# spacemeshos/go-spacemesh

Measured on AMD Instinct MI355X. Metric: post_labels_per_sec, higher is better.
Workload: dtype u32; 1 GPU; init-mainnet-scryptN8192-4units-256GiB-sink; step_labels=2097152, scrypt_n=8192, num_units=4, labels_per_unit=4294967296, parallelism=index-range shards x1, RCCL nonce min-reduce, vrf_nonce_found=True

## Files before the change

go-spacemesh_amd/csrc/engine.cpp:

```cpp
#include "../../include/spacemesh_post.h"

#include <hip/hip_runtime.h>

#include <fcntl.h>
#include <sys/stat.h>
#include <sys/types.h>
#include <unistd.h>

#include <algorithm>
#include <array>
#include <atomic>
#include <thread>
#include <chrono>
#include <cerrno>
#include <cstdio>
#include <cstdlib>
#include <cstring>
#include <functional>
#include <map>
#include <mutex>
#include <string>
#include <vector>

#include "crypto_host.h"
#include "kernel_args.h"
#include "post_common.h"

namespace {

thread_local std::string g_last_error;

void set_error(const std::string &e) { g_last_error = e; }

int hip_fail(const char *what, hipError_t err) {
  set_error(std::string(what) + ": " + hipGetErrorString(err));
  return err == hipErrorOutOfMemory ? POST_ERR_OOM : POST_ERR;
}

#define HIP_TRY(expr)                                                          \
  do {                                                                         \
    hipError_t _e = (expr);                                                    \
    if (_e != hipSuccess) return hip_fail(#expr, _e);                          \
  } while (0)

int require_gpu(uint32_t provider_id) {
  int count = 0;
  hipError_t e = hipGetDeviceCount(&count);
  if (e != hipSuccess || count == 0) {
    set_error("no HIP device available (the HIP engine has no CPU fallback)");
    return POST_ERR_NO_GPU;
  }
  if (provider_id >= (uint32_t)count) {
    set_error("provider id out of range");
    return POST_ERR_INVALID_ARGS;
  }
  e = hipSetDevice((int)provider_id);
  if (e != hipSuccess) return hip_fail("hipSetDevice", e);
  return POST_OK;
}

void load_commitment_words(const uint8_t c[32], uint32_t w[8]) {
  std::memcpy(w, c, 32);
}

void difficulty_to_be_words(const uint8_t d[32], uint32_t w[8]) {
  for (int i = 0; i < 8; i++)
    w[i] = ((uint32_t)d[4 * i] << 24) | ((uint32_t)d[4 * i + 1] << 16) |
           ((uint32_t)d[4 * i + 2] << 8) | d[4 * i + 3];
}

constexpr uint32_t THREADS = 256;
constexpr uint32_t CAND_CAP = 1 << 16;

uint32_t pick_gap_shift(uint32_t scrypt_n) {
  const char *env = getenv("POST_GAP_SHIFT");
  if (env) {
    uint32_t g = (uint32_t)atoi(env);
    while ((scrypt_n >> g) == 0) g--;
    return g;
  }
  return 0;
}

uint64_t prove_chunk_labels() {
  const uint64_t dflt = 1ull << 24;
  const char *env = getenv("POST_PROVE_CHUNK_LABELS");
  if (!env) return dflt;
  const long long v = strtoll(env, nullptr, 10);
  if (v <= 0 || (uint64_t)v >= dflt) return dflt;
  return v < 256 ? 256 : (uint64_t)v;
}

struct VerifyWorkspace {
  std::mutex mu;
  uint32_t *d_scratch = nullptr;
  size_t scratch_cap = 0;
  uint64_t *d_idx = nullptr;
  uint32_t *d_cid = nullptr;
  uint8_t *d_out = nullptr;
  uint32_t *d_xbuf = nullptr;
  size_t tasks_cap = 0;
  uint32_t *d_cm = nullptr;
  size_t cm_cap = 0;
  uint32_t *d_vrk = nullptr;
  uint8_t *d_half = nullptr;
  uint64_t *d_vdiff = nullptr;
  size_t proofs_cap = 0;
  uint8_t *d_pass = nullptr;
};
std::mutex g_vws_mu;
std::map<int, VerifyWorkspace *> g_vws;

VerifyWorkspace *get_verify_ws(int dev) {
  std::lock_guard<std::mutex> lk(g_vws_mu);
  auto it = g_vws.find(dev);
  if (it != g_vws.end()) return it->second;
  auto *w = new VerifyWorkspace();
  g_vws[dev] = w;
  return w;
}

int ws_reserve_proofs(VerifyWorkspace *w, size_t proofs) {
  if (proofs > w->proofs_cap) {
    size_t cap = std::max<size_t>(proofs, 1024);
    if (w->d_vrk) (void)hipFree(w->d_vrk);
    if (w->d_half) (void)hipFree(w->d_half);
    if (w->d_vdiff) (void)hipFree(w->d_vdiff);
    w->d_vrk = nullptr; w->d_half = nullptr; w->d_vdiff = nullptr;
    w->proofs_cap = 0;
    HIP_TRY(hipMalloc(&w->d_vrk, cap * 44 * 4));
    HIP_TRY(hipMalloc(&w->d_half, cap));
    HIP_TRY(hipMalloc(&w->d_vdiff, cap * 8));
    w->proofs_cap = cap;
  }
  return POST_OK;
}

int ws_reserve(VerifyWorkspace *w, size_t scratch_bytes, size_t tasks,
               size_t cm_words) {
  if (scratch_bytes > w->scratch_cap) {
    if (w->d_scratch) (void)hipFree(w->d_scratch);
    w->d_scratch = nullptr;
    w->scratch_cap = 0;
    HIP_TRY(hipMalloc(&w->d_scratch, scratch_bytes));
    w->scratch_cap = scratch_bytes;
  }
  if (tasks > w->tasks_cap) {
    size_t cap = std::max<size_t>(tasks, 4096);
    if (w->d_idx) (void)hipFree(w->d_idx);
    if (w->d_cid) (void)hipFree(w->d_cid);
    if (w->d_out) (void)hipFree(w->d_out);
    if (w->d_xbuf) (void)hipFree(w->d_xbuf);
    if (w->d_pass) (void)hipFree(w->d_pass);
    w->d_idx = nullptr; w->d_cid = nullptr; w->d_out = nullptr;
    w->d_xbuf = nullptr; w->d_pass = nullptr;
    w->tasks_cap = 0;
    HIP_TRY(hipMalloc(&w->d_idx, cap * 8));
    HIP_TRY(hipMalloc(&w->d_cid, cap * 4));
    HIP_TRY(hipMalloc(&w->d_out, cap * 32));
    HIP_TRY(hipMalloc(&w->d_xbuf, cap * 128));
    HIP_TRY(hipMalloc(&w->d_pass, cap));
    w->tasks_cap = cap;
  }
  if (cm_words > w->cm_cap) {
    size_t cap = std::max<size_t>(cm_words, 1024);
    if (w->d_cm) (void)hipFree(w->d_cm);
    w->d_cm = nullptr;
    w->cm_cap = 0;
    HIP_TRY(hipMalloc(&w->d_cm, cap * 4));
    w->cm_cap = cap;
  }
  return POST_OK;
}

struct DeviceTables {
  uint32_t *d_te = nullptr;
  uint8_t *d_sbox = nullptr;
};
std::mutex g_tables_mu;
std::map<int, DeviceTables> g_tables;

int get_aes_tables(int dev, DeviceTables &out) {
  std::lock_guard<std::mutex> lk(g_tables_mu);
  auto it = g_tables.find(dev);
  if (it != g_tables.end()) {
    out = it->second;
    return POST_OK;
  }
  static uint32_t te[1024];
  static uint8_t sbox[256];
  poste::aes128_tables(te, sbox);
  DeviceTables t;
  HIP_TRY(hipMalloc(&t.d_te, sizeof(te)));
  HIP_TRY(hipMalloc(&t.d_sbox, sizeof(sbox)));
  HIP_TRY(hipMemcpy(t.d_te, te, sizeof(te), hipMemcpyHostToDevice));
  HIP_TRY(hipMemcpy(t.d_sbox, sbox, sizeof(sbox), hipMemcpyHostToDevice));
  g_tables[dev] = t;
  out = t;
  return POST_OK;
}

}

extern "C" {

const char *post_last_error(void) { return g_last_error.c_str(); }

const char *post_engine_version(void) {
  return "spacemesh-post-hip 0.2 (gfx950)";
}


int post_providers(PostProvider *providers, uint32_t cap, uint32_t *count) {
  int n = 0;
  hipError_t e = hipGetDeviceCount(&n);
  if (e != hipSuccess) n = 0;
  *count = (uint32_t)n;
  for (uint32_t i = 0; i < (uint32_t)n && i < cap; i++) {
    hipDeviceProp_t prop;
    if (hipGetDeviceProperties(&prop, (int)i) != hipSuccess) continue;
    providers[i].id = i;
    std::snprintf(providers[i].model, sizeof(providers[i].model), "%s",
                  prop.name);
    providers[i].device_type = 0;
    providers[i].memory_bytes = prop.totalGlobalMem;
    providers[i].performance = 0;
  }
  return POST_OK;
}


struct PostInitSession {
  PostInitConfig cfg;
  std::string data_dir;
  uint64_t range_start = 0, range_end = 0;
  std::atomic<uint64_t> written{0};
  std::atomic<bool> cancel{false};
  uint8_t commitment[32];

  std::mutex nonce_mu;
  bool nonce_found = false;
  uint64_t nonce_idx = 0;
  uint8_t nonce_label[32];

  uint64_t lanes = 0;
  uint64_t batch_seq = 0;
  uint32_t gap_shift = 0;
  uint64_t batch = 0;
  uint32_t *d_scratch = nullptr;
  uint8_t *d_out = nullptr;
  uint8_t *d_all = nullptr;
  bool keep_all = false;
  PostVrfCandidate *d_cand = nullptr;
  unsigned int *d_cand_count = nullptr;
  uint32_t *d_xbuf = nullptr;
  uint8_t *h_batch = nullptr;
  hipStream_t stream = nullptr;
  hipEvent_t ev0 = nullptr, ev1 = nullptr;
  double last_kernel_ms = 0;

  int split_streams = 0;
  bool split_chain = false;
  uint64_t unit_cursor = 0;
  uint64_t split_batch_no = 0;
  uint32_t cand_cap = 0;
  uint8_t *d_out1 = nullptr;
  PostVrfCandidate *d_cand1 = nullptr;
  unsigned int *d_cand_count1 = nullptr;
  uint8_t *h_batch1 = nullptr;
  PostVrfCandidate *h_cand[2] = {nullptr, nullptr};
  unsigned int *h_cand_count = nullptr;
  hipStream_t stream_b = nullptr, stream_c = nullptr, copy_stream = nullptr;
  hipEvent_t ev_fill[4] = {nullptr, nullptr, nullptr, nullptr};
  hipEvent_t ev_tail[2][3] = {{nullptr, nullptr, nullptr},
                              {nullptr, nullptr, nullptr}};
  hipEvent_t ev_end[2] = {nullptr, nullptr}, ev_done[2] = {nullptr, nullptr};
  hipEvent_t ev_reset[2] = {nullptr, nullptr};

  ~PostInitSession() {
    if (stream) (void)hipStreamSynchronize(stream);
    if (stream_b) (void)hipStreamSynchronize(stream_b);
    if (stream_c) (void)hipStreamSynchronize(stream_c);
    if (copy_stream) (void)hipStreamSynchronize(copy_stream);
    for (int i = 0; i < 4; i++)
      if (ev_fill[i]) (void)hipEventDestroy(ev_fill[i]);
    for (int i = 0; i < 2; i++) {
      for (int k = 0; k < 3; k++)
        if (ev_tail[i][k]) (void)hipEventDestroy(ev_tail[i][k]);
      if (ev_reset[i]) (void)hipEventDestroy(ev_reset[i]);
      if (ev_end[i]) (void)hipEventDestroy(ev_end[i]);
      if (ev_done[i]) (void)hipEventDestroy(ev_done[i]);
      if (h_cand[i]) (void)hipHostFree(h_cand[i]);
    }
    if (stream_b) (void)hipStreamDestroy(stream_b);
    if (stream_c) (void)hipStreamDestroy(stream_c);
    if (copy_stream) (void)hipStreamDestroy(copy_stream);
    if (d_out1) (void)hipFree(d_out1);
    if (d_cand1) (void)hipFree(d_cand1);
    if (d_cand_count1) (void)hipFree(d_cand_count1);
    if (h_batch1) (void)hipHostFree(h_batch1);
    if (h_cand_count) (void)hipHostFree(h_cand_count);
    if (ev0) (void)hipEventDestroy(ev0);
    if (ev1) (void)hipEventDestroy(ev1);
    if (stream) (void)hipStreamDestroy(stream);
    if (d_scratch) (void)hipFree(d_scratch);
    if (d_out) (void)hipFree(d_out);
    if (d_all) (void)hipFree(d_all);
    if (d_cand) (void)hipFree(d_cand);
    if (d_cand_count) (void)hipFree(d_cand_count);
    if (d_xbuf) (void)hipFree(d_xbuf);
    if (h_batch) (void)hipHostFree(h_batch);
  }
};

static uint64_t existing_labels(const std::string &dir, uint64_t per_file,
                                uint64_t range_start, uint64_t range_total) {
  uint64_t done = 0;
  for (uint64_t pos = range_start; pos < range_start + range_total;) {
    uint64_t file_i = pos / per_file;
    uint64_t in_file = pos % per_file;
    uint64_t file_cap = std::min(per_file - in_file,
                                 range_start + range_total - pos);
    char path[4096];
    std::snprintf(path, sizeof path, "%s/postdata_%llu.bin", dir.c_str(),
                  (unsigned long long)file_i);
    FILE *f = std::fopen(path, "rb");
    if (!f) break;
    std::fseek(f, 0, SEEK_END);
    long sz = std::ftell(f);
    std::fclose(f);
    uint64_t labels_here = (uint64_t)(sz < 0 ? 0 : sz) / POST_LABEL_SIZE;
    if (in_file > labels_here) break;
    uint64_t usable = std::min(labels_here - in_file, file_cap);
    done += usable;
    pos += usable;
    if (usable < file_cap) break;
  }
  return done;
}

static int check_existing_metadata(PostInitSession *s);
static int write_metadata(PostInitSession *s);

int post_init_new(const PostInitConfig *cfg, PostInitSession **out) {
  if (!cfg || !out) {
    set_error("null args");
    return POST_ERR_INVALID_ARGS;
  }
  if (cfg->scrypt_n < 2 || (cfg->scrypt_n & (cfg->scrypt_n - 1))) {
    set_error("scrypt N must be a power of two >= 2");
    return POST_ERR_INVALID_ARGS;
  }
  int rc = require_gpu(cfg->provider_id);
  if (rc != POST_OK) return rc;

  struct Guard {
    PostInitSession *p;
    ~Guard() { delete p; }
  };
  auto *s = new PostInitSession();
  Guard guard{s};
  s->cfg = *cfg;
  if (cfg->data_dir) {
    s->data_dir = cfg->data_dir;
    std::string path;
    for (size_t i = 0; i <= s->data_dir.size(); i++) {
      if (i == s->data_dir.size() || s->data_dir[i] == '/') {
        path = s->data_dir.substr(0, i);
        if (!path.empty()) (void)::mkdir(path.c_str(), 0755);
      }
    }
    struct stat st;
    if (stat(s->data_dir.c_str(), &st) != 0 || !S_ISDIR(st.st_mode)) {
      set_error("cannot create data dir " + s->data_dir);
      return POST_ERR_IO;
    }
  }
  uint64_t total = (uint64_t)cfg->num_units * cfg->labels_per_unit;
  s->range_start = cfg->index_start;
  s->range_end = cfg->index_end ? cfg->index_end : total;
  if (s->range_end > total || s->range_start >= s->range_end) {
    set_error("bad index range");
    return POST_ERR_INVALID_ARGS;
  }
  poste::commitment(cfg->node_id, cfg->commitment_atx_id, s->commitment);

  s->gap_shift = pick_gap_shift(cfg->scrypt_n);
  size_t free_b = 0, total_b = 0;
  HIP_TRY(hipMemGetInfo(&free_b, &total_b));
  uint64_t budget = cfg->scratch_bytes
                        ? cfg->scratch_bytes
                        : (uint64_t)((double)free_b * 0.80);
  uint64_t per_lane = ((uint64_t)cfg->scrypt_n >> s->gap_shift) * 128;
  uint64_t lanes = budget / per_lane;
  uint64_t range = s->range_end - s->range_start;
  lanes = std::min<uint64_t>(lanes, std::max<uint64_t>(range, 64));
  lanes = std::min<uint64_t>(lanes,
                             poste_label_resident_slots(s->gap_shift));
  const char *const mx = getenv("POST_ROMIX_MIX");
  const bool want3 = !mx || !*mx || std::strcmp(mx, "free3") == 0;
  const uint64_t lane_round = want3 ? 64 : 128;
  lanes = (lanes / lane_round) * lane_round;
  if (lanes < 128) lanes = 128;
  if (lanes == 0) {
    set_error("not enough device memory for one scratch lane block");
    return POST_ERR_OOM;
  }
  s->lanes = lanes;
  s->batch = std::min<uint64_t>(range, lanes * 4);

  HIP_TRY(hipMalloc(&s->d_scratch, (size_t)lanes * per_lane));
  uint64_t keep_bytes = range * POST_LABEL_SIZE;
  s->keep_all = s->data_dir.empty() && keep_bytes <= (8ull << 30);
  if (s->keep_all) {
    HIP_TRY(hipMalloc(&s->d_all, (size_t)keep_bytes));
  }
  HIP_TRY(hipMalloc(&s->d_out, (size_t)s->batch * POST_LABEL_SIZE));
  s->cand_cap =
      (uint32_t)std::max<uint64_t>(CAND_CAP, s->batch / 64 + 16);
  HIP_TRY(hipMalloc(&s->d_cand, sizeof(PostVrfCandidate) * s->cand_cap));
  HIP_TRY(hipMalloc(&s->d_xbuf,
                    (size_t)std::max<uint64_t>(s->batch, lanes) * 128));
  HIP_TRY(hipMalloc(&s->d_cand_count, sizeof(unsigned int)));
  HIP_TRY(hipHostMalloc(&s->h_batch, (size_t)s->batch * POST_LABEL_SIZE));
  HIP_TRY(hipStreamCreate(&s->stream));

  {
    const bool lean = poste_label_romix_lean_ok(cfg->scrypt_n, s->gap_shift,
                                                lanes) != 0;
    if (!lean || (mx && std::strcmp(mx, "0") == 0))
      s->split_streams = 0;
    else if (mx && std::strcmp(mx, "seq") == 0)
      s->split_streams = 1;
    else if (want3 && lanes >= 192)
      s->split_streams = 3;
    else
      s->split_streams = lanes >= 128 ? 2 : 0;
    s->split_chain =
        s->split_streams == 2 && mx && std::strcmp(mx, "chain") == 0;
  }
  if (s->split_streams) {
    if (!s->keep_all)
      HIP_TRY(hipMalloc(&s->d_out1, (size_t)s->batch * POST_LABEL_SIZE));
    HIP_TRY(hipMalloc(&s->d_cand1, sizeof(PostVrfCandidate) * s->cand_cap));
    HIP_TRY(hipMalloc(&s->d_cand_count1, sizeof(unsigned int)));
    HIP_TRY(hipHostMalloc(&s->h_batch1, (size_t)s->batch * POST_LABEL_SIZE));
    HIP_TRY(hipHostMalloc(&s->h_cand_count, 2 * sizeof(unsigned int)));
    for (int i = 0; i < 2; i++) {
      HIP_TRY(hipHostMalloc(&s->h_cand[i],
                            sizeof(PostVrfCandidate) * s->cand_cap));
      HIP_TRY(hipEventCreate(&s->ev_end[i]));
      HIP_TRY(hipEventCreateWithFlags(&s->ev_done[i], hipEventDisableTiming));
      HIP_TRY(hipEventCreateWithFlags(&s->ev_reset[i],
                                      hipEventDisableTiming));
      for (int k = 0; k < s->split_streams; k++)
        HIP_TRY(hipEventCreateWithFlags(&s->ev_tail[i][k],
                                        hipEventDisableTiming));
    }
    if (s->split_chain)
      for (int i = 0; i < 4; i++)
        HIP_TRY(hipEventCreateWithFlags(&s->ev_fill[i],
                                        hipEventDisableTiming));
    if (s->split_streams >= 2) HIP_TRY(hipStreamCreate(&s->stream_b));
    if (s->split_streams >= 3) HIP_TRY(hipStreamCreate(&s->stream_c));
    HIP_TRY(hipStreamCreate(&s->copy_stream));
  }

  if (!s->data_dir.empty()) {
    rc = check_existing_metadata(s);
    if (rc != POST_OK) return rc;
    rc = write_metadata(s);
    if (rc != POST_OK) return rc;
    uint64_t per_file = std::max<uint64_t>(
        1, s->cfg.max_file_size / POST_LABEL_SIZE);
    s->written = existing_labels(s->data_dir, per_file, s->range_start, range);
  }
  guard.p = nullptr;
  *out = s;
  return POST_OK;
}

uint64_t post_init_num_labels_written(const PostInitSession *s) {
  return s ? s->written.load() : 0;
}

void post_init_cancel(PostInitSession *s) {
  if (s) s->cancel = true;
}

int post_init_nonce(const PostInitSession *s, uint64_t *index,
                    uint8_t label[32]) {
  auto *m = const_cast<PostInitSession *>(s);
  std::lock_guard<std::mutex> lk(m->nonce_mu);
  if (!s->nonce_found) return POST_ERR;
  *index = s->nonce_idx;
  std::memcpy(label, s->nonce_label, 32);
  return POST_OK;
}

static int write_batch_files(PostInitSession *s, uint64_t pos, uint64_t count,
                             const uint8_t *host_labels) {
  uint64_t per_file =
      std::max<uint64_t>(1, s->cfg.max_file_size / POST_LABEL_SIZE);
  uint64_t off = 0;
  while (off < count) {
    uint64_t gpos = pos + off;
    uint64_t file_i = gpos / per_file;
    uint64_t in_file = gpos % per_file;
    uint64_t take = std::min(per_file - in_file, count - off);
    char path[4096];
    std::snprintf(path, sizeof path, "%s/postdata_%llu.bin",
                  s->data_dir.c_str(), (unsigned long long)file_i);
    FILE *f = std::fopen(path, "r+b");
    if (!f) f = std::fopen(path, "w+b");
    if (!f) {
      set_error(std::string("cannot open ") + path);
      return POST_ERR_IO;
    }
    std::fseek(f, (long)(in_file * POST_LABEL_SIZE), SEEK_SET);
    size_t wr = std::fwrite(host_labels + off * POST_LABEL_SIZE,
                            POST_LABEL_SIZE, take, f);
    std::fclose(f);
    if (wr != take) {
      set_error("short write");
      return POST_ERR_IO;
    }
    off += take;
  }
  return POST_OK;
}

static void b64(const uint8_t *in, size_t n, std::string &out) {
  static const char t[] =
      "ABCDEFGHIJKLMNOPQRSTUVWXYZabcdefghijklmnopqrstuvwxyz0123456789+/";
  for (size_t i = 0; i < n; i += 3) {
    uint32_t v = (uint32_t)in[i] << 16;
    if (i + 1 < n) v |= (uint32_t)in[i + 1] << 8;
    if (i + 2 < n) v |= in[i + 2];
    out += t[(v >> 18) & 63];
    out += t[(v >> 12) & 63];
    out += i + 1 < n ? t[(v >> 6) & 63] : '=';
    out += i + 2 < n ? t[v & 63] : '=';
  }
}

static bool b64_decode(const std::string &in, uint8_t *out, size_t want) {
  static int8_t rev[256];
  static bool init = false;
  if (!init) {
    static const char t[] =
        "ABCDEFGHIJKLMNOPQRSTUVWXYZabcdefghijklmnopqrstuvwxyz0123456789+/";
    for (int i = 0; i < 256; i++) rev[i] = -1;
    for (int i = 0; i < 64; i++) rev[(uint8_t)t[i]] = (int8_t)i;
    init = true;
  }
  size_t n = 0;
  uint32_t acc = 0;
  int bits = 0;
  for (char c : in) {
    if (c == '=') break;
    int8_t v = rev[(uint8_t)c];
    if (v < 0) return false;
    acc = (acc << 6) | (uint32_t)v;
    bits += 6;
    if (bits >= 8) {
      bits -= 8;
      if (n >= want) return false;
      out[n++] = (uint8_t)(acc >> bits);
    }
  }
  return n == want;
}

static bool md_find_string(const std::string &j, const char *key,
                           std::string &out) {
  std::string pat = std::string("\"") + key + "\": \"";
  size_t p = j.find(pat);
  if (p == std::string::npos) return false;
  p += pat.size();
  size_t e = j.find('"', p);
  if (e == std::string::npos) return false;
  out = j.substr(p, e - p);
  return true;
}

static bool md_find_u64(const std::string &j, const char *key,
                        uint64_t &out) {
  std::string pat = std::string("\"") + key + "\": ";
  size_t p = j.find(pat);
  if (p == std::string::npos) return false;
  out = strtoull(j.c_str() + p + pat.size(), nullptr, 10);
  return true;
}

static int check_existing_metadata(PostInitSession *s) {
  char path[4096];
  std::snprintf(path, sizeof path, "%s/postdata_metadata.json",
                s->data_dir.c_str());
  FILE *f = std::fopen(path, "rb");
  if (!f) return POST_OK;
  std::string j;
  char buf[4096];
  size_t rd;
  while ((rd = std::fread(buf, 1, sizeof buf, f)) > 0) j.append(buf, rd);
  std::fclose(f);
  std::string nid_b64, atx_b64, want_nid, want_atx;
  b64(s->cfg.node_id, 32, want_nid);
  b64(s->cfg.commitment_atx_id, 32, want_atx);
  uint64_t lpu = 0, n = 0;
  if (md_find_string(j, "NodeId", nid_b64) && nid_b64 != want_nid) {
    set_error("data dir belongs to a different node id (postdata_metadata"
              ".json mismatch)");
    return POST_ERR_INVALID_ARGS;
  }
  if (md_find_string(j, "CommitmentAtxId", atx_b64) &&
      atx_b64 != want_atx) {
    set_error("data dir was initialized for a different commitment ATX");
    return POST_ERR_INVALID_ARGS;
  }
  if (md_find_u64(j, "LabelsPerUnit", lpu) &&
      lpu != s->cfg.labels_per_unit) {
    set_error("data dir was initialized with a different LabelsPerUnit");
    return POST_ERR_INVALID_ARGS;
  }
  if (md_find_u64(j, "N", n) && n != s->cfg.scrypt_n) {
    set_error("data dir was initialized with different scrypt params");
    return POST_ERR_INVALID_ARGS;
  }
  uint64_t nonce_idx = 0;
  std::string nv_b64;
  if (md_find_u64(j, "Nonce", nonce_idx) &&
      md_find_string(j, "NonceValue", nv_b64)) {
    uint8_t label[32];
    if (!b64_decode(nv_b64, label, 32)) {
      set_error("postdata_metadata.json NonceValue is not 32 base64 bytes");
      return POST_ERR_INVALID_ARGS;
    }
    std::lock_guard<std::mutex> lk(s->nonce_mu);
    s->nonce_found = true;
    s->nonce_idx = nonce_idx;
    std::memcpy(s->nonce_label, label, 32);
  }
  return POST_OK;
}

static int write_metadata(PostInitSession *s) {
  std::string nid, atx, nv;
  b64(s->cfg.node_id, 32, nid);
  b64(s->cfg.commitment_atx_id, 32, atx);
  char path[4096];
  std::snprintf(path, sizeof path, "%s/postdata_metadata.json",
                s->data_dir.c_str());
  FILE *f = std::fopen(path, "w");
  if (!f) {
    set_error("cannot write metadata");
    return POST_ERR_IO;
  }
  std::fprintf(f,
               "{\n  \"NodeId\": \"%s\",\n  \"CommitmentAtxId\": \"%s\",\n"
               "  \"LabelsPerUnit\": %llu,\n  \"NumUnits\": %u,\n"
               "  \"MaxFileSize\": %llu,\n  \"Scrypt\": {\"N\": %u, \"R\": 1,"
               " \"P\": 1}",
               nid.c_str(), atx.c_str(),
               (unsigned long long)s->cfg.labels_per_unit, s->cfg.num_units,
               (unsigned long long)s->cfg.max_file_size, s->cfg.scrypt_n);
  std::lock_guard<std::mutex> lk(s->nonce_mu);
  if (s->nonce_found) {
    b64(s->nonce_label, 32, nv);
    std::fprintf(f, ",\n  \"Nonce\": %llu,\n  \"NonceValue\": \"%s\"",
                 (unsigned long long)s->nonce_idx, nv.c_str());
  }
  std::fprintf(f, "\n}\n");
  std::fclose(f);
  return POST_OK;
}

static int init_step_split(PostInitSession *s, uint64_t max_labels,
                           uint64_t *done) {
  const int ns = s->split_streams;
  const uint64_t unit = s->lanes / (uint64_t)ns / 64 * 64;
  hipStream_t st[3] = {s->stream, s->stream_b, s->stream_c};
  uint8_t *const d_outs[2] = {s->d_out, s->d_out1};
  uint8_t *const h_batches[2] = {s->h_batch, s->h_batch1};
  PostVrfCandidate *const d_cands[2] = {s->d_cand, s->d_cand1};
  unsigned int *const d_counts[2] = {s->d_cand_count, s->d_cand_count1};

  auto drain = [&] {
    for (int k = 0; k < ns; k++) (void)hipStreamSynchronize(st[k]);
    (void)hipStreamSynchronize(s->copy_stream);
  };
#define SPLIT_TRY(expr)                                                        \
  do {                                                                         \
    hipError_t _e = (expr);                                                    \
    if (_e != hipSuccess) {                                                    \
      drain();                                                                 \
      return hip_fail(#expr, _e);                                              \
    }                                                                          \
  } while (0)

  LabelKernelArgs args;
  std::memset(&args, 0, sizeof(args));
  load_commitment_words(s->commitment, args.commitment_le);
  args.scrypt_n = s->cfg.scrypt_n;
  args.gap_shift = s->gap_shift;
  args.scratch = s->d_scratch;
  args.scratch_lanes = s->lanes;
  args.has_difficulty = 1;
  args.cand_cap = s->cand_cap;
  RomixPhaseArgs ph;
  std::memset(&ph, 0, sizeof(ph));
  ph.scratch = s->d_scratch;
  ph.scratch_lanes = s->lanes;
  ph.slot_count = unit;
  ph.scrypt_n = s->cfg.scrypt_n;

  uint8_t cur_difficulty[32];
  std::memset(cur_difficulty, 0xff, 32);
  {
    std::lock_guard<std::mutex> lk(s->nonce_mu);
    if (s->nonce_found) std::memcpy(cur_difficulty, s->nonce_label, 32);
  }
  const char *sp_env = getenv("POST_SELFCHECK_PERIOD");
  long selfcheck_period = sp_env ? strtol(sp_env, nullptr, 10) : 1;
  if (selfcheck_period < 1) selfcheck_period = 1;

  if (!s->ev0) SPLIT_TRY(hipEventCreate(&s->ev0));
  s->last_kernel_ms = 0;

  struct Batch {
    uint64_t pos = 0, count = 0;
    uint32_t max_cand = 0;
    int set = 0;
    bool live = false;
  };
  uint64_t issued = 0;
  int last_set = -1;

  auto issue = [&](Batch &b) -> int {
    b.set = (int)(s->split_batch_no++ & 1);
    b.max_cand = 0;
    uint8_t *out =
        s->keep_all ? s->d_all + b.pos * POST_LABEL_SIZE : d_outs[b.set];
    args.cand = d_cands[b.set];
    args.cand_count = d_counts[b.set];
    difficulty_to_be_words(cur_difficulty, args.difficulty_be);
    const int k0 = (int)(s->unit_cursor % (uint64_t)ns);
    SPLIT_TRY(hipMemsetAsync(d_counts[b.set], 0, sizeof(unsigned int),
                             st[k0]));
    if (ns > 1) SPLIT_TRY(hipEventRecord(s->ev_reset[b.set], st[k0]));
    const uint64_t nunits = (b.count + unit - 1) / unit;
    const uint64_t per = ((b.count + nunits - 1) / nunits + 63) / 64 * 64;
    bool used[3] = {false, false, false};
    for (uint64_t off = 0; off < b.count; off += per) {
      const int k = (int)(s->unit_cursor % (uint64_t)ns);
      const uint64_t c = std::min(per, b.count - off);
      const uint32_t blocks = (uint32_t)((c + 63) / 64);
      args.start = s->range_start + b.pos + off;
      args.count = c;
      args.xbuf = s->d_xbuf + (uint64_t)k * unit * 32;
      args.out = out + off * POST_LABEL_SIZE;
      ph.xbuf = args.xbuf;
      ph.slot_base = (uint64_t)k * unit;
      ph.count = c;
      if (issued == 0) SPLIT_TRY(hipEventRecord(s->ev0, st[k]));
      SPLIT_TRY(poste_launch_label_prologue(&args, blocks, st[k]));
      if (s->split_chain && issued > 0)
        SPLIT_TRY(hipStreamWaitEvent(
            st[k], s->ev_fill[(s->unit_cursor - 1) & 3], 0));
      SPLIT_TRY(poste_launch_romix_fill(&ph, st[k]));
      if (s->split_chain)
        SPLIT_TRY(hipEventRecord(s->ev_fill[s->unit_cursor & 3], st[k]));
      SPLIT_TRY(poste_launch_romix_mix(&ph, st[k]));
      if (k != k0 && !used[k])
        SPLIT_TRY(hipStreamWaitEvent(st[k], s->ev_reset[b.set], 0));
      SPLIT_TRY(poste_launch_label_tail(&args, blocks, st[k]));
      b.max_cand += blocks;
      used[k] = true;
      s->unit_cursor++;
      issued++;
    }
    for (int k = 0; k < ns; k++) {
      if (!used[k]) continue;
      SPLIT_TRY(hipEventRecord(s->ev_tail[b.set][k], st[k]));
      SPLIT_TRY(hipStreamWaitEvent(s->copy_stream, s->ev_tail[b.set][k], 0));
    }
    SPLIT_TRY(hipEventRecord(s->ev_end[b.set], s->copy_stream));
    SPLIT_TRY(hipMemcpyAsync(h_batches[b.set], out,
                             b.count * POST_LABEL_SIZE, hipMemcpyDeviceToHost,
                             s->copy_stream));
    SPLIT_TRY(hipMemcpyAsync(s->h_cand_count + b.set, d_counts[b.set],
                             sizeof(unsigned int), hipMemcpyDeviceToHost,
                             s->copy_stream));
    b.max_cand = std::min(b.max_cand, s->cand_cap);
    SPLIT_TRY(hipMemcpyAsync(s->h_cand[b.set], d_cands[b.set],
                             sizeof(PostVrfCandidate) * b.max_cand,
                             hipMemcpyDeviceToHost, s->copy_stream));
    SPLIT_TRY(hipEventRecord(s->ev_done[b.set], s->copy_stream));
    last_set = b.set;
    b.live = true;
    return POST_OK;
  };

  auto process = [&](Batch &b) -> int {
    b.live = false;
    const bool do_selfcheck =
        (s->batch_seq++ % (uint64_t)selfcheck_period) == 0;
    const uint64_t probe = b.count / 2;
    uint8_t ref[32];
    const int ref_rc =
        do_selfcheck
            ? poste::host_label(s->commitment, s->range_start + b.pos + probe,
                                s->cfg.scrypt_n, ref)
            : 0;
    SPLIT_TRY(hipEventSynchronize(s->ev_done[b.set]));
    const unsigned int take = std::min(s->h_cand_count[b.set], b.max_cand);
    const PostVrfCandidate *cands = s->h_cand[b.set];
    bool nonce_improved = false;
    if (take > 0) {
      std::lock_guard<std::mutex> lk(s->nonce_mu);
      for (unsigned int i = 0; i < take; i++) {
        uint8_t lab[32];
        for (int k = 0; k < 8; k++) {
          uint32_t w = cands[i].label_be[k];
          lab[4 * k] = (uint8_t)(w >> 24);
          lab[4 * k + 1] = (uint8_t)(w >> 16);
          lab[4 * k + 2] = (uint8_t)(w >> 8);
          lab[4 * k + 3] = (uint8_t)w;
        }
        int c = std::memcmp(lab, cur_difficulty, 32);
        if (!s->nonce_found || c < 0 ||
            (c == 0 && cands[i].index < s->nonce_idx)) {
          s->nonce_found = true;
          s->nonce_idx = cands[i].index;
          std::memcpy(s->nonce_label, lab, 32);
          std::memcpy(cur_difficulty, lab, 32);
          nonce_improved = true;
        }
      }
    }
    int rc = POST_OK;
    if (nonce_improved && !s->data_dir.empty()) rc = write_metadata(s);
    if (rc == POST_OK && ref_rc != 0) {
      set_error("host reference label failed");
      rc = POST_ERR;
    }
    if (rc == POST_OK && do_selfcheck &&
        std::memcmp(ref, h_batches[b.set] + probe * POST_LABEL_SIZE,
                    POST_LABEL_SIZE) != 0) {
      set_error("reference label mismatch: device labels diverge from the "
                "host reference (ErrReferenceLabelMismatch)");
      rc = POST_ERR;
    }
    if (rc == POST_OK && !s->data_dir.empty())
      rc = write_batch_files(s, s->range_start + b.pos, b.count,
                             h_batches[b.set]);
    if (rc != POST_OK) {
      drain();
      return rc;
    }
    s->written.store(b.pos + b.count);
    *done += b.count;
    return POST_OK;
  };

  const uint64_t range = s->range_end - s->range_start;
  uint64_t pos = s->written.load();
  const uint64_t target = std::min(range, pos + max_labels);
  Batch inflight[2];
  int cur = 0;
  bool cancelled = false;
  while (pos < target) {
    if (s->cancel.load()) {
      cancelled = true;
      break;
    }
    Batch &b = inflight[cur];
    b.pos = pos;
    b.count = std::min(s->batch, target - pos);
    int rc = issue(b);
    if (rc != POST_OK) return rc;
    pos += b.count;
    if (inflight[cur ^ 1].live) {
      rc = process(inflight[cur ^ 1]);
      if (rc != POST_OK) return rc;
    }
    cur ^= 1;
  }
  if (inflight[cur ^ 1].live) {
    int rc = process(inflight[cur ^ 1]);
    if (rc != POST_OK) return rc;
  }
  drain();
  if (last_set >= 0) {
    float ms = 0;
    (void)hipEventElapsedTime(&ms, s->ev0, s->ev_end[last_set]);
    s->last_kernel_ms = ms;
  }
#undef SPLIT_TRY
  return cancelled ? POST_ERR_CANCELLED : POST_OK;
}

int post_init_step(PostInitSession *s, uint64_t max_labels, uint64_t *done) {
  if (!s || !done) return POST_ERR_INVALID_ARGS;
  *done = 0;
  int rc = require_gpu(s->cfg.provider_id);
  if (rc != POST_OK) return rc;
  if (s->split_streams) return init_step_split(s, max_labels, done);

  LabelKernelArgs args;
  std::memset(&args, 0, sizeof(args));
  load_commitment_words(s->commitment, args.commitment_le);
  args.scrypt_n = s->cfg.scrypt_n;
  args.gap_shift = s->gap_shift;
  args.xbuf = s->d_xbuf;
  args.out_full = 0;
  args.scratch = s->d_scratch;
  args.scratch_lanes = s->lanes;
  args.indices = nullptr;
  args.commit_ids = nullptr;
  args.commitments = nullptr;
  args.has_difficulty = 1;
  args.cand = s->d_cand;
  args.cand_count = s->d_cand_count;
  args.cand_cap = s->cand_cap;

  uint8_t cur_difficulty[32];
  std::memset(cur_difficulty, 0xff, 32);
  {
    std::lock_guard<std::mutex> lk(s->nonce_mu);
    if (s->nonce_found) std::memcpy(cur_difficulty, s->nonce_label, 32);
  }

  const uint32_t blocks = (uint32_t)(s->lanes / 64);
  std::vector<PostVrfCandidate> cands(s->cand_cap);

  if (!s->ev0) {
    HIP_TRY(hipEventCreate(&s->ev0));
    HIP_TRY(hipEventCreate(&s->ev1));
  }
  s->last_kernel_ms = 0;

  uint64_t range = s->range_end - s->range_start;
  uint64_t pos = s->written.load();
  uint64_t target = std::min(range, pos + max_labels);
  while (pos < target) {
    if (s->cancel.load()) return POST_ERR_CANCELLED;
    uint64_t count = std::min(s->batch, target - pos);
    args.start = s->range_start + pos;
    args.count = count;
    args.out = s->keep_all ? s->d_all + pos * POST_LABEL_SIZE : s->d_out;
    difficulty_to_be_words(cur_difficulty, args.difficulty_be);
    unsigned int zero = 0;
    HIP_TRY(hipMemcpyAsync(s->d_cand_count, &zero, sizeof(zero),
                           hipMemcpyHostToDevice, s->stream));
    HIP_TRY(hipEventRecord(s->ev0, s->stream));
    HIP_TRY(poste_launch_label_kernel(&args, blocks, s->stream));
    HIP_TRY(hipEventRecord(s->ev1, s->stream));
    HIP_TRY(hipMemcpyAsync(s->h_batch, args.out, count * POST_LABEL_SIZE,
                           hipMemcpyDeviceToHost, s->stream));
    unsigned int n_cand = 0;
    HIP_TRY(hipMemcpyAsync(&n_cand, s->d_cand_count, sizeof(n_cand),
                           hipMemcpyDeviceToHost, s->stream));
    const char *sp_env = getenv("POST_SELFCHECK_PERIOD");
    long selfcheck_period = sp_env ? strtol(sp_env, nullptr, 10) : 1;
    if (selfcheck_period < 1) selfcheck_period = 1;
    const bool do_selfcheck = (s->batch_seq++ % (uint64_t)selfcheck_period)
                              == 0;
    const uint64_t probe = count / 2;
    uint8_t ref[32];
    const int ref_rc =
        do_selfcheck ? poste::host_label(s->commitment, args.start + probe,
                                         s->cfg.scrypt_n, ref)
                     : 0;
    HIP_TRY(hipStreamSynchronize(s->stream));
    bool nonce_improved = false;
    if (n_cand > 0) {
      unsigned int take = std::min(n_cand, s->cand_cap);
      HIP_TRY(hipMemcpy(cands.data(), s->d_cand,
                        sizeof(PostVrfCandidate) * take,
                        hipMemcpyDeviceToHost));
      std::lock_guard<std::mutex> lk(s->nonce_mu);
      for (unsigned int i = 0; i < take; i++) {
        uint8_t lab[32];
        for (int k = 0; k < 8; k++) {
          uint32_t w = cands[i].label_be[k];
          lab[4 * k] = (uint8_t)(w >> 24);
          lab[4 * k + 1] = (uint8_t)(w >> 16);
          lab[4 * k + 2] = (uint8_t)(w >> 8);
          lab[4 * k + 3] = (uint8_t)w;
        }
        int c = std::memcmp(lab, cur_difficulty, 32);
        if (!s->nonce_found || c < 0 ||
            (c == 0 && cands[i].index < s->nonce_idx)) {
          s->nonce_found = true;
          s->nonce_idx = cands[i].index;
          std::memcpy(s->nonce_label, lab, 32);
          std::memcpy(cur_difficulty, lab, 32);
          nonce_improved = true;
        }
      }
    }
    if (nonce_improved && !s->data_dir.empty()) {
      rc = write_metadata(s);
      if (rc != POST_OK) return rc;
    }

    if (ref_rc != 0) {
      set_error("host reference label failed");
      return POST_ERR;
    }
    if (do_selfcheck &&
        std::memcmp(ref, s->h_batch + probe * POST_LABEL_SIZE,
                    POST_LABEL_SIZE) != 0) {
      set_error("reference label mismatch: device labels diverge from the "
                "host reference (ErrReferenceLabelMismatch)");
      return POST_ERR;
    }

    if (!s->data_dir.empty()) {
      rc = write_batch_files(s, s->range_start + pos, count, s->h_batch);
      if (rc != POST_OK) return rc;
    }
    float ms = 0;
    (void)hipEventElapsedTime(&ms, s->ev0, s->ev1);
    s->last_kernel_ms += ms;
    pos += count;
    s->written.store(pos);
    *done += count;
  }
  return POST_OK;
}

double post_init_last_kernel_ms(const PostInitSession *s) {
  return s ? s->last_kernel_ms : 0.0;
}

static int nonce_only_batch(PostInitSession *s, uint64_t gstart,
                            uint64_t count) {
  LabelKernelArgs args;
  std::memset(&args, 0, sizeof(args));
  load_commitment_words(s->commitment, args.commitment_le);
  args.scrypt_n = s->cfg.scrypt_n;
  args.gap_shift = s->gap_shift;
  args.xbuf = s->d_xbuf;
  args.scratch = s->d_scratch;
  args.scratch_lanes = s->lanes;
  args.start = gstart;
  args.count = count;
  args.out = nullptr;
  args.has_difficulty = 1;
  args.cand = s->d_cand;
  args.cand_count = s->d_cand_count;
  args.cand_cap = s->cand_cap;
  uint8_t cur[32];
  std::memset(cur, 0xff, 32);
  {
    std::lock_guard<std::mutex> lk(s->nonce_mu);
    if (s->nonce_found) std::memcpy(cur, s->nonce_label, 32);
  }
  difficulty_to_be_words(cur, args.difficulty_be);
  unsigned int zero = 0;
  HIP_TRY(hipMemcpy(s->d_cand_count, &zero, sizeof(zero),
                    hipMemcpyHostToDevice));
  HIP_TRY(poste_launch_label_kernel(&args, (uint32_t)(s->lanes / 64),
                                    s->stream));
  HIP_TRY(hipStreamSynchronize(s->stream));
  unsigned int n_cand = 0;
  HIP_TRY(hipMemcpy(&n_cand, s->d_cand_count, sizeof(n_cand),
                    hipMemcpyDeviceToHost));
  if (n_cand > 0) {
    unsigned int take = std::min(n_cand, s->cand_cap);
    std::vector<PostVrfCandidate> cands(take);
    HIP_TRY(hipMemcpy(cands.data(), s->d_cand,
                      sizeof(PostVrfCandidate) * take,
                      hipMemcpyDeviceToHost));
    bool improved = false;
    {
      std::lock_guard<std::mutex> lk(s->nonce_mu);
      for (unsigned int i = 0; i < take; i++) {
        uint8_t lab[32];
        for (int k = 0; k < 8; k++) {
          uint32_t w = cands[i].label_be[k];
          lab[4 * k] = (uint8_t)(w >> 24);
          lab[4 * k + 1] = (uint8_t)(w >> 16);
          lab[4 * k + 2] = (uint8_t)(w >> 8);
          lab[4 * k + 3] = (uint8_t)w;
        }
        int c = s->nonce_found ? std::memcmp(lab, s->nonce_label, 32) : -1;
        if (c < 0 || (c == 0 && cands[i].index < s->nonce_idx)) {
          s->nonce_found = true;
          s->nonce_idx = cands[i].index;
          std::memcpy(s->nonce_label, lab, 32);
          improved = true;
        }
      }
    }
    if (improved && !s->data_dir.empty()) {
      int rc = write_metadata(s);
      if (rc != POST_OK) return rc;
    }
  }
  return POST_OK;
}

int post_init_run(PostInitSession *s) {
  if (!s) return POST_ERR_INVALID_ARGS;
  uint64_t range = s->range_end - s->range_start;
  while (s->written.load() < range) {
    uint64_t done = 0;
    int rc = post_init_step(s, s->batch * 8, &done);
    if (rc != POST_OK) return rc;
    if (done == 0) break;
  }

  uint64_t total = (uint64_t)s->cfg.num_units * s->cfg.labels_per_unit;
  if (s->range_start == 0 && s->range_end == total) {
    uint8_t diff[32];
    poste::vrf_difficulty(total, diff);
    for (uint64_t ext = total; ext < 2 * total; ext += s->batch) {
      {
        std::lock_guard<std::mutex> lk(s->nonce_mu);
        if (s->nonce_found &&
            std::memcmp(s->nonce_label, diff, 32) < 0)
          break;
      }
      if (s->cancel.load()) return POST_ERR_CANCELLED;
      int rc = nonce_only_batch(s, ext, std::min(s->batch, 2 * total - ext));
      if (rc != POST_OK) return rc;
    }
  }

  if (!s->data_dir.empty()) return write_metadata(s);
  return POST_OK;
}

int post_init_copy_labels(const PostInitSession *s, uint64_t first,
                          uint64_t count, uint8_t *out_host) {
  if (!s || !out_host) return POST_ERR_INVALID_ARGS;
  if (!s->keep_all) {
    set_error("labels were not kept on device (file mode or large range)");
    return POST_ERR_INVALID_ARGS;
  }
  if (first + count > s->range_end - s->range_start) {
    set_error("range out of bounds");
    return POST_ERR_INVALID_ARGS;
  }
  HIP_TRY(hipMemcpy(out_host, s->d_all + first * POST_LABEL_SIZE,
                    count * POST_LABEL_SIZE, hipMemcpyDeviceToHost));
  return POST_OK;
}

void post_init_free(PostInitSession *s) { delete s; }


int post_benchmark(uint32_t provider_id, uint32_t scrypt_n,
                   uint64_t *labels_per_sec) {
  int rc = require_gpu(provider_id);
  if (rc != POST_OK) return rc;
  PostInitConfig cfg;
  std::memset(&cfg, 0, sizeof(cfg));
  std::memset(cfg.node_id, 0xA5, 32);
  std::memset(cfg.commitment_atx_id, 0x5A, 32);
  cfg.num_units = 1;
  cfg.labels_per_unit = 1ull << 18;
  cfg.max_file_size = 1ull << 40;
  cfg.scrypt_n = scrypt_n;
  cfg.provider_id = provider_id;
  cfg.scratch_bytes = 8ull << 30;
  PostInitSession *s = nullptr;
  rc = post_init_new(&cfg, &s);
// ... 2006 lines not shown
```

Before: 2.243 million labels/s.

## Move label prologue and tail onto a service stream with double-buffered xbuf

The label prologue and tail kernels leave the per-lane streams and run on one service stream, which also takes the candidate reset and the device-to-host copies. Prologues are queued one unit ahead into a double-buffered xbuf, and per-unit events tie them to the romix fill/mix stages. The aim is to keep the romix streams busy with fill/mix only and to hide prologue and tail work behind them. In exchange the xbuf doubles in size, there are many more events, and all prologue and tail work is serialized on a single stream, which could become the bottleneck.

```diff
diff --git a/go-spacemesh_amd/csrc/engine.cpp b/go-spacemesh_amd/csrc/engine.cpp
--- a/go-spacemesh_amd/csrc/engine.cpp
+++ b/go-spacemesh_amd/csrc/engine.cpp
@@ -261,6 +261,7 @@
 
   int split_streams = 0;
   bool split_chain = false;
+  uint64_t split_unit = 0;
   uint64_t unit_cursor = 0;
   uint64_t split_batch_no = 0;
   uint32_t cand_cap = 0;
@@ -270,31 +271,31 @@
   uint8_t *h_batch1 = nullptr;
   PostVrfCandidate *h_cand[2] = {nullptr, nullptr};
   unsigned int *h_cand_count = nullptr;
-  hipStream_t stream_b = nullptr, stream_c = nullptr, copy_stream = nullptr;
+  hipStream_t stream_b = nullptr, stream_c = nullptr;
+  hipStream_t service_stream = nullptr;
   hipEvent_t ev_fill[4] = {nullptr, nullptr, nullptr, nullptr};
-  hipEvent_t ev_tail[2][3] = {{nullptr, nullptr, nullptr},
-                              {nullptr, nullptr, nullptr}};
   hipEvent_t ev_end[2] = {nullptr, nullptr}, ev_done[2] = {nullptr, nullptr};
-  hipEvent_t ev_reset[2] = {nullptr, nullptr};
+  std::vector<hipEvent_t> ev_pro, ev_mix;
 
   ~PostInitSession() {
     if (stream) (void)hipStreamSynchronize(stream);
     if (stream_b) (void)hipStreamSynchronize(stream_b);
     if (stream_c) (void)hipStreamSynchronize(stream_c);
-    if (copy_stream) (void)hipStreamSynchronize(copy_stream);
+    if (service_stream) (void)hipStreamSynchronize(service_stream);
     for (int i = 0; i < 4; i++)
       if (ev_fill[i]) (void)hipEventDestroy(ev_fill[i]);
+    for (hipEvent_t e : ev_pro)
+      if (e) (void)hipEventDestroy(e);
+    for (hipEvent_t e : ev_mix)
+      if (e) (void)hipEventDestroy(e);
     for (int i = 0; i < 2; i++) {
-      for (int k = 0; k < 3; k++)
-        if (ev_tail[i][k]) (void)hipEventDestroy(ev_tail[i][k]);
-      if (ev_reset[i]) (void)hipEventDestroy(ev_reset[i]);
       if (ev_end[i]) (void)hipEventDestroy(ev_end[i]);
       if (ev_done[i]) (void)hipEventDestroy(ev_done[i]);
       if (h_cand[i]) (void)hipHostFree(h_cand[i]);
     }
     if (stream_b) (void)hipStreamDestroy(stream_b);
     if (stream_c) (void)hipStreamDestroy(stream_c);
-    if (copy_stream) (void)hipStreamDestroy(copy_stream);
+    if (service_stream) (void)hipStreamDestroy(service_stream);
     if (d_out1) (void)hipFree(d_out1);
     if (d_cand1) (void)hipFree(d_cand1);
     if (d_cand_count1) (void)hipFree(d_cand_count1);
@@ -420,7 +421,7 @@
       (uint32_t)std::max<uint64_t>(CAND_CAP, s->batch / 64 + 16);
   HIP_TRY(hipMalloc(&s->d_cand, sizeof(PostVrfCandidate) * s->cand_cap));
   HIP_TRY(hipMalloc(&s->d_xbuf,
-                    (size_t)std::max<uint64_t>(s->batch, lanes) * 128));
+                    (size_t)std::max<uint64_t>(s->batch, 2 * lanes) * 128));
   HIP_TRY(hipMalloc(&s->d_cand_count, sizeof(unsigned int)));
   HIP_TRY(hipHostMalloc(&s->h_batch, (size_t)s->batch * POST_LABEL_SIZE));
   HIP_TRY(hipStreamCreate(&s->stream));
@@ -451,11 +452,16 @@
                             sizeof(PostVrfCandidate) * s->cand_cap));
       HIP_TRY(hipEventCreate(&s->ev_end[i]));
       HIP_TRY(hipEventCreateWithFlags(&s->ev_done[i], hipEventDisableTiming));
-      HIP_TRY(hipEventCreateWithFlags(&s->ev_reset[i],
-                                      hipEventDisableTiming));
-      for (int k = 0; k < s->split_streams; k++)
-        HIP_TRY(hipEventCreateWithFlags(&s->ev_tail[i][k],
-                                        hipEventDisableTiming));
+    }
+    s->split_unit = lanes / (uint64_t)s->split_streams / 64 * 64;
+    const size_t n_ev =
+        2 * (size_t)((s->batch + s->split_unit - 1) / s->split_unit) +
+        (size_t)s->split_streams;
+    s->ev_pro.assign(n_ev, nullptr);
+    s->ev_mix.assign(n_ev, nullptr);
+    for (size_t i = 0; i < n_ev; i++) {
+      HIP_TRY(hipEventCreateWithFlags(&s->ev_pro[i], hipEventDisableTiming));
+      HIP_TRY(hipEventCreateWithFlags(&s->ev_mix[i], hipEventDisableTiming));
     }
     if (s->split_chain)
       for (int i = 0; i < 4; i++)
@@ -463,7 +469,7 @@
                                         hipEventDisableTiming));
     if (s->split_streams >= 2) HIP_TRY(hipStreamCreate(&s->stream_b));
     if (s->split_streams >= 3) HIP_TRY(hipStreamCreate(&s->stream_c));
-    HIP_TRY(hipStreamCreate(&s->copy_stream));
+    HIP_TRY(hipStreamCreate(&s->service_stream));
   }
 
   if (!s->data_dir.empty()) {
@@ -678,8 +684,10 @@
 static int init_step_split(PostInitSession *s, uint64_t max_labels,
                            uint64_t *done) {
   const int ns = s->split_streams;
-  const uint64_t unit = s->lanes / (uint64_t)ns / 64 * 64;
+  const uint64_t unit = s->split_unit;
+  const uint64_t n_ev = s->ev_pro.size();
   hipStream_t st[3] = {s->stream, s->stream_b, s->stream_c};
+  hipStream_t const svc = s->service_stream;
   uint8_t *const d_outs[2] = {s->d_out, s->d_out1};
   uint8_t *const h_batches[2] = {s->h_batch, s->h_batch1};
   PostVrfCandidate *const d_cands[2] = {s->d_cand, s->d_cand1};
@@ -687,7 +695,7 @@
 
   auto drain = [&] {
     for (int k = 0; k < ns; k++) (void)hipStreamSynchronize(st[k]);
-    (void)hipStreamSynchronize(s->copy_stream);
+    (void)hipStreamSynchronize(svc);
   };
 #define SPLIT_TRY(expr)                                                        \
   do {                                                                         \
@@ -736,6 +744,42 @@
   uint64_t issued = 0;
   int last_set = -1;
 
+  const uint64_t range = s->range_end - s->range_start;
+  uint64_t pos = s->written.load();
+  const uint64_t target = std::min(range, pos + max_labels);
+
+  auto unit_labels = [&](uint64_t batch_count) -> uint64_t {
+    const uint64_t nunits = (batch_count + unit - 1) / unit;
+    return ((batch_count + nunits - 1) / nunits + 63) / 64 * 64;
+  };
+  auto xbuf_of = [&](uint64_t u) -> uint32_t * {
+    const uint64_t k = u % (uint64_t)ns, half = (u / (uint64_t)ns) & 1;
+    return s->d_xbuf + (2 * k + half) * unit * 32;
+  };
+
+  LabelKernelArgs pargs = args;
+  uint64_t la_unit = s->unit_cursor;
+  uint64_t la_pos = pos, la_count = 0, la_per = 0, la_off = 0;
+  auto queue_prologue = [&]() -> int {
+    if (la_off >= la_count) {
+      la_pos += la_count;
+      la_count = std::min(s->batch, target - la_pos);
+      if (la_count == 0) return POST_OK;
+      la_per = unit_labels(la_count);
+      la_off = 0;
+    }
+    const uint64_t c = std::min(la_per, la_count - la_off);
+    pargs.start = s->range_start + la_pos + la_off;
+    pargs.count = c;
+    pargs.xbuf = xbuf_of(la_unit);
+    SPLIT_TRY(poste_launch_label_prologue(&pargs, (uint32_t)((c + 63) / 64),
+                                          svc));
+    SPLIT_TRY(hipEventRecord(s->ev_pro[la_unit % n_ev], svc));
+    la_off += la_per;
+    la_unit++;
+    return POST_OK;
+  };
+
   auto issue = [&](Batch &b) -> int {
     b.set = (int)(s->split_batch_no++ & 1);
     b.max_cand = 0;
@@ -744,58 +788,56 @@
     args.cand = d_cands[b.set];
     args.cand_count = d_counts[b.set];
     difficulty_to_be_words(cur_difficulty, args.difficulty_be);
-    const int k0 = (int)(s->unit_cursor % (uint64_t)ns);
-    SPLIT_TRY(hipMemsetAsync(d_counts[b.set], 0, sizeof(unsigned int),
-                             st[k0]));
-    if (ns > 1) SPLIT_TRY(hipEventRecord(s->ev_reset[b.set], st[k0]));
-    const uint64_t nunits = (b.count + unit - 1) / unit;
-    const uint64_t per = ((b.count + nunits - 1) / nunits + 63) / 64 * 64;
-    bool used[3] = {false, false, false};
+    if (issued == 0) {
+      SPLIT_TRY(hipEventRecord(s->ev0, svc));
+      for (int k = 0; k < ns; k++) {
+        const int rc = queue_prologue();
+        if (rc != POST_OK) return rc;
+      }
+    }
+    const uint64_t per = unit_labels(b.count);
     for (uint64_t off = 0; off < b.count; off += per) {
-      const int k = (int)(s->unit_cursor % (uint64_t)ns);
+      const uint64_t u = s->unit_cursor;
+      const int k = (int)(u % (uint64_t)ns);
       const uint64_t c = std::min(per, b.count - off);
       const uint32_t blocks = (uint32_t)((c + 63) / 64);
+      ph.xbuf = xbuf_of(u);
+      ph.slot_base = (uint64_t)k * unit;
+      ph.count = c;
+      SPLIT_TRY(hipStreamWaitEvent(st[k], s->ev_pro[u % n_ev], 0));
+      if (s->split_chain && issued > 0)
+        SPLIT_TRY(hipStreamWaitEvent(st[k], s->ev_fill[(u - 1) & 3], 0));
+      SPLIT_TRY(poste_launch_romix_fill(&ph, st[k]));
+      if (s->split_chain) SPLIT_TRY(hipEventRecord(s->ev_fill[u & 3], st[k]));
+      SPLIT_TRY(poste_launch_romix_mix(&ph, st[k]));
+      SPLIT_TRY(hipEventRecord(s->ev_mix[u % n_ev], st[k]));
+      const int rc = queue_prologue();
+      if (rc != POST_OK) return rc;
+      if (off == 0)
+        SPLIT_TRY(hipMemsetAsync(d_counts[b.set], 0, sizeof(unsigned int),
+                                 svc));
+      SPLIT_TRY(hipStreamWaitEvent(svc, s->ev_mix[u % n_ev], 0));
       args.start = s->range_start + b.pos + off;
       args.count = c;
-      args.xbuf = s->d_xbuf + (uint64_t)k * unit * 32;
+      args.xbuf = ph.xbuf;
       args.out = out + off * POST_LABEL_SIZE;
-      ph.xbuf = args.xbuf;
-      ph.slot_base = (uint64_t)k * unit;
-      ph.count = c;
-      if (issued == 0) SPLIT_TRY(hipEventRecord(s->ev0, st[k]));
-      SPLIT_TRY(poste_launch_label_prologue(&args, blocks, st[k]));
-      if (s->split_chain && issued > 0)
-        SPLIT_TRY(hipStreamWaitEvent(
-            st[k], s->ev_fill[(s->unit_cursor - 1) & 3], 0));
-      SPLIT_TRY(poste_launch_romix_fill(&ph, st[k]));
-      if (s->split_chain)
-        SPLIT_TRY(hipEventRecord(s->ev_fill[s->unit_cursor & 3], st[k]));
-      SPLIT_TRY(poste_launch_romix_mix(&ph, st[k]));
-      if (k != k0 && !used[k])
-        SPLIT_TRY(hipStreamWaitEvent(st[k], s->ev_reset[b.set], 0));
-      SPLIT_TRY(poste_launch_label_tail(&args, blocks, st[k]));
+      SPLIT_TRY(poste_launch_label_tail(&args, blocks, svc));
       b.max_cand += blocks;
-      used[k] = true;
       s->unit_cursor++;
       issued++;
     }
-    for (int k = 0; k < ns; k++) {
-      if (!used[k]) continue;
-      SPLIT_TRY(hipEventRecord(s->ev_tail[b.set][k], st[k]));
-      SPLIT_TRY(hipStreamWaitEvent(s->copy_stream, s->ev_tail[b.set][k], 0));
-    }
-    SPLIT_TRY(hipEventRecord(s->ev_end[b.set], s->copy_stream));
+    SPLIT_TRY(hipEventRecord(s->ev_end[b.set], svc));
     SPLIT_TRY(hipMemcpyAsync(h_batches[b.set], out,
                              b.count * POST_LABEL_SIZE, hipMemcpyDeviceToHost,
-                             s->copy_stream));
+                             svc));
     SPLIT_TRY(hipMemcpyAsync(s->h_cand_count + b.set, d_counts[b.set],
                              sizeof(unsigned int), hipMemcpyDeviceToHost,
-                             s->copy_stream));
+                             svc));
     b.max_cand = std::min(b.max_cand, s->cand_cap);
     SPLIT_TRY(hipMemcpyAsync(s->h_cand[b.set], d_cands[b.set],
                              sizeof(PostVrfCandidate) * b.max_cand,
-                             hipMemcpyDeviceToHost, s->copy_stream));
-    SPLIT_TRY(hipEventRecord(s->ev_done[b.set], s->copy_stream));
+                             hipMemcpyDeviceToHost, svc));
+    SPLIT_TRY(hipEventRecord(s->ev_done[b.set], svc));
     last_set = b.set;
     b.live = true;
     return POST_OK;
@@ -863,9 +905,6 @@
     return POST_OK;
   };
 
-  const uint64_t range = s->range_end - s->range_start;
-  uint64_t pos = s->written.load();
-  const uint64_t target = std::min(range, pos + max_labels);
   Batch inflight[2];
   int cur = 0;
   bool cancelled = false;
```

Measured after the change: 2.247 million labels/s, median of 2. No clear change (+0.2%).
